# hasindu2008/sigfish

Measured on AMD Instinct MI355X. Metric: reads/s (sDTW alignment stage: nCoV-2019 R9 DNA, -q 250, both strands), higher is better.
Workload: dtype f32

## Files before the change

### include/sigfish_amd.h

```cpp
#ifndef SIGFISH_AMD_H
#define SIGFISH_AMD_H

#include <stddef.h>
#include <stdint.h>

#ifdef __cplusplus
extern "C" {
#endif

#define SFA_VERSION "0.1.0"

#define SFA_RNA 0x001
#define SFA_DTW 0x002
#define SFA_INV 0x004
#define SFA_REF 0x010
#define SFA_END 0x020

enum {
    SFA_OK = 0,
    SFA_EINVAL = -1,
    SFA_ENODEV = -2,
    SFA_ENOMEM = -3,
    SFA_ERANGE = -4,
    SFA_EKERNEL = -5
// ... 21 lines not shown
    uint8_t pad;
} sfa_result_t;

typedef struct {
    uint64_t start;
    float length;
    float mean;
    float stdv;
} sfa_event_t;

typedef struct sfa_ctx sfa_ctx_t;

typedef struct {
    double fill_ms;
    double trace_ms;
    double finalize_ms;
    double total_ms;
    int64_t cells;
    int64_t fill_launches;
    int64_t ckpt_interval;
    int64_t ckpt_bytes;
    int64_t n_tasks;
    int64_t n_chunks;
    int64_t n_segments;
    int64_t segment_reruns;
    double events_ms;
    double normalise_ms;
    int64_t non_finite_reads;
    double decode_ms;
    int64_t blow5_fallbacks;
    int64_t lds_ckpt;
    int64_t trace_margin;
    int64_t fused_trace;
} sfa_profile_t;

typedef struct {
    int32_t n_quads;
    int32_t n_chunks;
    int32_t n_classes;
    int32_t max_rows_per_lane;
    int32_t ckpt_interval;
    int32_t trace_margin;
    int64_t ckpt_bytes;
    int64_t n_tasks;
    int32_t max_lanes_per_read;
    int32_t lane_widening;
} sfa_plan_info_t;

int sfa_init(sfa_ctx_t **ctx, const sfa_ref_t *ref, uint32_t flag, int device);

int sfa_init_devices(sfa_ctx_t **ctx, const sfa_ref_t *ref, uint32_t flag, const int *devices, int n_devices);

int sfa_n_devices(sfa_ctx_t *ctx);

int sfa_align_batch(sfa_ctx_t *ctx, const float *queries, const int64_t *q_off, int32_t n_reads, sfa_result_t *out);

int sfa_align_batch_device(sfa_ctx_t *ctx, const float *d_queries, const int64_t *q_off, int32_t n_reads,
                           sfa_result_t *d_out, int sync);

int sfa_submit_batch(sfa_ctx_t *ctx, const float *queries, const int64_t *q_off, int32_t n_reads);
int sfa_wait_batch(sfa_ctx_t *ctx, sfa_result_t *out, int32_t n_reads);

int sfa_secondary_rows(sfa_ctx_t *ctx, sfa_result_t *sec, int32_t n_reads);

int sfa_event_maps(sfa_ctx_t *ctx, const sfa_result_t *rows, const int32_t *read_of_row, int32_t n_rows, const int64_t *map_off,
                   int32_t *pairs, int32_t *n_on_host);
// ... 119 lines not shown
```

### sigfish_amd/_lib.py

```python
import ctypes as C
import os

HERE = os.path.dirname(os.path.abspath(__file__))
LIB_PATH = os.environ.get("SFA_LIB") or os.path.join(HERE, "lib", "libsigfish_amd.so")

f32p = C.POINTER(C.c_float)
i32p = C.POINTER(C.c_int32)
i64p = C.POINTER(C.c_int64)


class SfaRef(C.Structure):
    _fields_ = [("num_ref", C.c_int32), ("ref_lengths", i32p), ("ref_st_offset", i32p),
                ("forward", C.POINTER(f32p)), ("reverse", C.POINTER(f32p))]


class SfaResult(C.Structure):
    _fields_ = [("rid", C.c_int32), ("pos_st", C.c_int32), ("pos_end", C.c_int32), ("score", C.c_float),
                ("score2", C.c_float), ("strand", C.c_int8), ("mapq", C.c_uint8), ("valid", C.c_uint8),
                ("pad", C.c_uint8)]


class SfaProfile(C.Structure):
    _fields_ = [("fill_ms", C.c_double), ("trace_ms", C.c_double), ("finalize_ms", C.c_double),
                ("total_ms", C.c_double), ("cells", C.c_int64), ("fill_launches", C.c_int64),
                ("ckpt_interval", C.c_int64), ("ckpt_bytes", C.c_int64), ("n_tasks", C.c_int64),
                ("n_chunks", C.c_int64), ("n_segments", C.c_int64), ("segment_reruns", C.c_int64),
                ("events_ms", C.c_double), ("normalise_ms", C.c_double), ("non_finite_reads", C.c_int64), ("decode_ms", C.c_double), ("blow5_fallbacks", C.c_int64), ("lds_ckpt", C.c_int64), ("trace_margin", C.c_int64), ("fused_trace", C.c_int64)]


class SfaPlanInfo(C.Structure):
    _fields_ = [("n_quads", C.c_int32), ("n_chunks", C.c_int32), ("n_classes", C.c_int32),
                ("max_rows_per_lane", C.c_int32), ("ckpt_interval", C.c_int32), ("trace_margin", C.c_int32),
                ("ckpt_bytes", C.c_int64), ("n_tasks", C.c_int64), ("max_lanes_per_read", C.c_int32),
                ("lane_widening", C.c_int32)]


class SfaQueryInfo(C.Structure):
    _fields_ = [("n_events", C.c_int64), ("qstart", C.c_int64), ("qend", C.c_int64), ("start_raw_idx", C.c_uint64),
                ("end_raw_idx", C.c_uint64), ("status", C.c_int32), ("pad", C.c_int32)]


class SfaReadHead(C.Structure):
    _fields_ = [("read_id", C.c_char * 128), ("id_len", C.c_int32), ("pad", C.c_int32), ("n_samples", C.c_int64),
                ("digitisation", C.c_double), ("offset", C.c_double), ("range", C.c_double), ("record_bytes", C.c_int64)]


class SfaEvent(C.Structure):
    _fields_ = [("start", C.c_uint64), ("length", C.c_float), ("mean", C.c_float), ("stdv", C.c_float)]


SYMBOLS = ["sfa_init", "sfa_init_devices", "sfa_n_devices", "sfa_align_batch", "sfa_submit_batch", "sfa_wait_batch", "sfa_align_batch_device", "sfa_align_events", "sfa_align_raw", "sfa_align_raw_ex", "sfa_align_blow5", "sfa_inflate_zlib_device", "sfa_pinned_alloc", "sfa_pinned_free", "sfa_sync",
           "sfa_get_profile", "sfa_stream", "sfa_set_option", "sfa_plan_batch", "sfa_destroy", "sfa_last_error", "sfa_version", "sfa_build_id", "sfa_gen_ref_record",
           "sfa_znormalise", "sfa_paf_row", "sfa_sam_row", "sfa_paf_row_ex", "sfa_sam_row_ex", "sfa_secondary_rows", "sfa_event_maps", "sfa_sam_row_from_map", "sfa_r2qevent_map", "sfa_detect_events", "sfa_select_query", "sfa_detect_query_start", "sfa_set_pore", "sfa_read_kmer_model",
           "sfa_blow5_open", "sfa_blow5_attr", "sfa_blow5_next", "sfa_blow5_close", "sfa_blow5_select_shard", "sfa_blow5_select_records", "sfa_inflate_zlib", "sfa_inflate_zlib_pair", "sfa_device_memory"]

_lib = None


def load():
    global _lib
# ... 80 lines not shown
```

### sigfish_amd/csrc/sdtw_kernels.hpp

```cpp
#pragma once

#include <hip/hip_runtime.h>
#include <stdint.h>

namespace sfa {

constexpr int kRefPad = 128;
#ifndef SFA_STEPS_PER_LOAD
#define SFA_STEPS_PER_LOAD 4
#endif
#ifndef SFA_FILL_WAVES
#define SFA_FILL_WAVES 6
#endif
#ifndef SFA_FILL32_WAVES
#define SFA_FILL32_WAVES 4
#endif
#ifndef SFA_LCK_WAVES
#define SFA_LCK_WAVES 4
#endif
#ifndef SFA_TRACE_WAVES
#define SFA_TRACE_WAVES 4
#endif
constexpr int kStepsPerLoad = SFA_STEPS_PER_LOAD;
constexpr int kSpanBuckets = 32;
// ... 19 lines not shown
    const int32_t *quad_qlen;
    const float *ref;
    const int64_t *job_off;
    const int32_t *job_len;
    const int32_t *chunk_begin;
    const int32_t *job_ck_off;
    float *ck;
    float *p_best;
    int32_t *p_end;
    int32_t *p_job;
    float *p_second;
    int32_t *w_job;
    int32_t *w_end;
    float *w_score;
    ClassDesc cls[kMaxClasses];
    int32_t n_cls;
    int32_t n_chunks;
    int32_t n_tasks;
    int32_t rev_query;
    int32_t ck_shift;
    int32_t trace_margin;
    int32_t n_reads_total;
    int32_t n_seg;
    int32_t warm_windows;
    int32_t n_jobs;
    int32_t verify_planes;
    float *verify;
    int32_t *seg_fail;
    float *best_rec;
    int32_t *best_e;
    unsigned *g_best;
    int32_t *w_chunk;
    int32_t best_planes;
    int32_t coarse_every;
    int32_t lck_shift;
    const struct DpArgs *self;
    unsigned *ticket;
    int32_t *quad_done;
    int32_t n_quads_total;
    const int32_t *job_contig;
    const int8_t *job_strand;
    const int32_t *ref_len;
    const int32_t *ref_st_offset;
    const uint8_t *bad;
    struct ResultRow *out;
    unsigned *span_hist;
    int32_t prio_unit;
    unsigned *started;
    unsigned *err;
    long long spin_limit;
    int32_t debug_drop_quad;
    unsigned long long *task_times;
    int32_t *p_top5;
};

constexpr int kSimdSlots = 16384;
__device__ __forceinline__ unsigned simd_position() {
    const unsigned hw = __builtin_amdgcn_s_getreg((31 << 11) | (0 << 6) | 4);
    const unsigned xcc = __builtin_amdgcn_s_getreg((3 << 11) | (0 << 6) | 20);
    const unsigned simd = (hw >> 4) & 3, cu = (hw >> 8) & 15, sh = (hw >> 12) & 1, se = (hw >> 13) & 7;
    return ((((xcc & 15) * 8 + se) * 2 + sh) * 16 + cu) * 4 + simd;
}

__device__ __forceinline__ void drain_stores() { asm volatile("s_waitcnt vmcnt(0)" ::: "memory"); }
template <int OFF>
__device__ __forceinline__ void store_wt(const float *base, const float v) {
    static_assert(OFF >= 0 && OFF < 4096, "12-bit immediate");
    asm volatile("global_store_dword %0, %1, off offset:%2 sc1" ::"v"(base), "v"(v), "n"(OFF) : "memory");
// ... 230 lines not shown
}

template <int R>
__device__ __forceinline__ void load_query_rows(float (&x)[R], const DpArgs &a, int read, int qlen, int g, int g0 = 0) {
    const float *q = a.queries + a.q_off[read >= 0 ? read : 0];
#pragma unroll
    for (int r = 0; r < R; ++r) {
        const int i = (g - g0) * R + r;
        const int src = a.rev_query ? (qlen - 1 - i) : i;
        x[r] = (read >= 0 && i >= 0 && i < qlen) ? q[src] : 0.0f;
    }
}

struct LdsRows {
    typedef __attribute__((address_space(3))) volatile float lds_vf;
    float *p;
    __device__ __forceinline__ float operator[](const int r) const { return *((lds_vf *)(p + r * 64)); }
    template <int R>
    __device__ __forceinline__ void load(const DpArgs &a, int read, int qlen, int g, int g0) {
        const float *q = a.queries + a.q_off[read >= 0 ? read : 0];
        for (int r = 0; r < R; ++r) {
            const int i = (g - g0) * R + r;
            const int src = a.rev_query ? (qlen - 1 - i) : i;
            *((lds_vf *)(p + r * 64)) = (read >= 0 && i >= 0 && i < qlen) ? q[src] : 0.0f;
        }
    }
};

__device__ __forceinline__ int sweep_begin(int lq) { return lq - ((lq + kStepsPerLoad - 1) & ~(kStepsPerLoad - 1)); }

template <int R>
__device__ __forceinline__ constexpr int ck_planes() { return R + 2; }

constexpr int kLdsCkShift = 9;
constexpr int kLdsCkPlanes = 17;
struct LdsCkpt {
    float *buf;
    int count;
    int e0, e1;
    float *rec;
    int32_t *rec_e;
    unsigned *g_best;
    __device__ __forceinline__ void begin_job() { count = 0; }
    template <int R, typename CV>
    __device__ __forceinline__ void snapshot(const CV &cv, float dprev, int e) {
        count += 1;
        float *b = buf + (count & 1) * (kLdsCkPlanes * 64);
#pragma unroll
        for (int r = 0; r < R; ++r) b[r * 64] = cv[r];
        b[R * 64] = dprev;
        if (count & 1)
            e1 = e;
        else
            e0 = e;
    }
    template <int R, int L, bool WT = false>
    __device__ __forceinline__ void save(unsigned long long improved, float wmin, int e_ws, int margin, int lq, int job, int shift) {
        const int lane = threadIdx.x & 63;
        const int owner_lane = (lane & ~(L - 1)) + lq;
        const bool mine = (improved >> owner_lane) & 1;
        const unsigned wb = __float_as_uint(__shfl(wmin, owner_lane));
        unsigned old = 0;
        if (mine && lane == owner_lane) old = atomicMin(g_best, wb);
        old = __shfl(old, owner_lane);
        if (!(mine && wb <= old)) return;
        const int from = e_ws - margin - 3;
        const int kk = from > 0 ? (from >> shift) : 0;
        if (kk > 0) {
            const float *b = buf + (kk & 1) * (kLdsCkPlanes * 64);
#pragma unroll
            for (int r = 0; r <= R; ++r) {
                if (WT)
                    __hip_atomic_store(rec + r * 64, b[r * 64], __ATOMIC_RELAXED, __HIP_MEMORY_SCOPE_AGENT);
                else
                    rec[r * 64] = b[r * 64];
            }
        }
        if (lane == owner_lane) {
            const int ev = kk > 0 ? ((kk & 1) ? e1 : e0) : -1;
            if (WT)
                __hip_atomic_store(rec_e + lane / L, ev, __ATOMIC_RELAXED, __HIP_MEMORY_SCOPE_AGENT);
            else
                rec_e[lane / L] = ev;
        }
        (void)job;
    }
};

template <int R, bool STD, int RQ, bool LCK = false, int L = 16, bool WT = false, bool SEC = false>
__device__ __forceinline__ void sweep_job(const DpArgs &a, const float *yp, const int rlen, const int qlen, const int lq, const int rq,
                                          const int t_begin, const float (&x)[R], const bool lane0, Exchange &xc, Top2 &top,
                                          const int job, float *ckp, const int T, IssuePriority &pr, const MixedQuad &mq,
                                          LdsCkpt *lck = nullptr, const bool owner = false, int *t5 = nullptr) {
    constexpr bool TRACK = false;
    typename Vec<float, R>::type cv;
    typename Vec<int, R>::type sv;
#pragma unroll
    for (int r = 0; r < R; ++r) {
        cv[r] = INFINITY;
        sv[r] = 0;
    }
    float dprev = INFINITY;
    int sdprev = 0;
    xc.template set_boundary<TRACK>(lane0, 0.0f);

    int e = 0;
    int ck_next = T ? T : 0x7fffffff;
    const int ck_last = T ? ((rlen > 4 ? rlen - 4 : 0) >> a.ck_shift) << a.ck_shift : 0;
    constexpr bool SNAP = LCK && !STD;
    if (SNAP) {
        lck->begin_job();
        ck_next = 1 << a.lck_shift;
    }
    auto maybe_checkpoint = [&]() {
        if (SNAP) {
            if (e >= ck_next) {
                lck->template snapshot<R>(cv, dprev, e);
                ck_next += 1 << a.lck_shift;
                if (T && (lck->count & (a.coarse_every - 1)) == 0 && (lck->count << a.lck_shift) <= ck_last) {
                    if (WT) {
#pragma unroll
                        for (int r = 0; r < R; ++r) __hip_atomic_store(ckp + r * 64, static_cast<float>(cv[r]), __ATOMIC_RELAXED, __HIP_MEMORY_SCOPE_AGENT);
                        __hip_atomic_store(ckp + R * 64, dprev, __ATOMIC_RELAXED, __HIP_MEMORY_SCOPE_AGENT);
                        __hip_atomic_store(ckp + (R + 1) * 64, __int_as_float(e), __ATOMIC_RELAXED, __HIP_MEMORY_SCOPE_AGENT);
                    } else {
#pragma unroll
                        for (int r = 0; r < R; ++r) ckp[r * 64] = cv[r];
                        ckp[R * 64] = dprev;
                        ckp[(R + 1) * 64] = __int_as_float(e);
                    }
                    ckp += ck_planes<R>() * 64;
                }
            }
        } else if (T) {
            if (e >= ck_next && ck_next <= ck_last) {
                if (WT) {
                    store_record_wt<R>(ckp, cv, dprev, e);
                } else {
#pragma unroll
                    for (int r = 0; r < R; ++r) ckp[r * 64] = cv[r];
                    ckp[R * 64] = dprev;
                    ckp[(R + 1) * 64] = __int_as_float(e);
                }
                ckp += ck_planes<R>() * 64;
                ck_next += T;
            }
        }
    };

#define SFA_DP_STEP(YV, U)                                                                                                   \
    do {                                                                                                                     \
        if constexpr (STD) {                                                                                                 \
            if (e >= kStepsPerLoad)                                                                                          \
                dp_step<R, TRACK, STD, int, false>(cv, sv, dprev, sdprev, x, (YV), t_begin + e + (U), lane0, xc);            \
            else                                                                                                             \
                dp_step<R, TRACK, STD, int, true>(cv, sv, dprev, sdprev, x, (YV), t_begin + e + (U), lane0, xc);             \
        } else {                                                                                                             \
            dp_step<R, TRACK, STD, int>(cv, sv, dprev, sdprev, x, (YV), t_begin + e + (U), lane0, xc);                       \
        }                                                                                                                    \
    } while (0)
    float4u ycur = *reinterpret_cast<const float4u *>(yp);
    const int e_main = lq - t_begin;
    for (; e < e_main; e += kStepsPerLoad) {
        const float4u ynext = *reinterpret_cast<const float4u *>(yp + e + kStepsPerLoad);
        maybe_checkpoint();
#pragma unroll
        for (int u = 0; u < kStepsPerLoad; ++u) SFA_DP_STEP(ycur.v[u], u);
        ycur = ynext;
    }
    int jqv = 0;
    constexpr bool MIX = !STD;
    constexpr bool CELL = CellFromFill<R, STD>::value;
    constexpr int NS = 64 / L;
    const int my_slot = (threadIdx.x & 63) / L;
    int q_s[NS], ws_s[NS], we_s[NS];
#pragma unroll
    for (int sl = 0; sl < NS; ++sl) {
        q_s[sl] = MIX ? __builtin_amdgcn_readlane(mq.myq, sl * L) : qlen;
        ws_s[sl] = 0;
        we_s[sl] = min(q_s[sl], rlen);
    }
    float wmin = INFINITY;
    int wpos = CELL ? 0 : -1;
    for (int col = 0; col < rlen;) {
        pr.at_window(col);
        int nxt = we_s[0];
#pragma unroll
        for (int sl = 1; sl < NS; ++sl) nxt = min(nxt, we_s[sl]);
        const int wl = STD ? rlen : nxt - col;
        const int nb = wl >> 2, rm = wl & 3;
        auto track = [&]() {
            const float cl = (RQ >= 0) ? static_cast<float>(cv[RQ >= 0 ? RQ : 0]) : static_cast<float>(cv[rq]);
            if (!CELL) {
                wmin = fminf(wmin, cl);
            } else {
                const bool lt = cl < wmin;
                wmin = lt ? cl : wmin;
                wpos = lt ? jqv : wpos;
                jqv += 1;
            }
        };
        auto block = [&](const float4u &yv) {
            maybe_checkpoint();
#pragma unroll
            for (int u = 0; u < kStepsPerLoad; ++u) {
                SFA_DP_STEP(yv.v[u], u);
                if (!STD) track();
            }
            e += kStepsPerLoad;
        };
        int b = 0;
        for (; R < 32 && b + 1 < nb; b += 2) {
            const float4u yb = *reinterpret_cast<const float4u *>(yp + e + kStepsPerLoad);
            block(ycur);
            ycur = *reinterpret_cast<const float4u *>(yp + e + kStepsPerLoad);
            block(yb);
        }
        for (; b < nb; ++b) {
            const float4u yb = *reinterpret_cast<const float4u *>(yp + e + kStepsPerLoad);
            block(ycur);
            ycur = yb;
        }
        if (rm) {
            const float4u ynext = *reinterpret_cast<const float4u *>(yp + e + rm);
            maybe_checkpoint();
#pragma unroll
            for (int u = 0; u < kStepsPerLoad - 1; ++u) {
                if (u < rm) {
                    SFA_DP_STEP(ycur.v[u], u);
                    if (!STD) track();
                }
            }
            e += rm;
            ycur = ynext;
        }
        if (MIX) {
            unsigned long long endmask = 0;
            int wsl = ws_s[0];
#pragma unroll
            for (int sl = 0; sl < NS; ++sl) {
                const unsigned long long lanes_of_slot = (L == 64) ? ~0ull : (((1ull << (L & 63)) - 1) << ((sl * L) & 63));
                if (we_s[sl] == nxt) endmask |= lanes_of_slot;
                if (sl > 0) wsl = (my_slot == sl) ? ws_s[sl] : wsl;
            }
            const bool ending = (endmask >> (threadIdx.x & 63)) & 1;
            const bool became_best = top.offer_if(ending, wmin, CELL ? wpos : wsl, job);
            if constexpr (SEC) {
                if (ending && owner) top5_offer(t5, wmin, CELL ? wpos : wsl, job);
            }
            if (LCK) {
                const unsigned long long improved = __ballot(became_best && owner);
                if (improved) lck->template save<R, L, WT>(improved, wmin, wsl + e_main, a.trace_margin, lq, job, a.lck_shift);
            }
            wmin = ending ? INFINITY : wmin;
            if (CELL) wpos = ending ? nxt : wpos;
#pragma unroll
            for (int sl = 0; sl < NS; ++sl) {
                if (we_s[sl] == nxt) {
                    ws_s[sl] = nxt;
                    we_s[sl] = min(nxt + q_s[sl], rlen);
                }
            }
        } else {
            const float cl = (RQ >= 0) ? static_cast<float>(cv[RQ >= 0 ? RQ : 0]) : static_cast<float>(cv[rq]);
            top.offer(cl, rlen - 1, job);
            if constexpr (SEC) {
                if (owner) top5_offer(t5, cl, rlen - 1, job);
            }
        }
        col += wl;
    }
    pr.remaining -= rlen;
#undef SFA_DP_STEP
}

template <int R, bool STD, bool LCK = false, int L = 16, bool WT = false, int I = 0, bool SEC = false>
__device__ __forceinline__ void sweep_dispatch(const DpArgs &a, const float *yp, int rlen, int qlen, int lq, int rq, int t_begin,
                                               const float (&x)[R], bool lane0, Exchange &xc, Top2 &top, int job, float *ckp, int T,
                                               IssuePriority &pr, const MixedQuad &mq, LdsCkpt *lck = nullptr, bool owner = false,
                                               int *t5 = nullptr) {
    if constexpr (STD || R > 16) {
        sweep_job<R, STD, -1, LCK, L, WT, SEC>(a, yp, rlen, qlen, lq, rq, t_begin, x, lane0, xc, top, job, ckp, T, pr, mq, lck, owner, t5);
    } else {
        if (rq == I) {
            sweep_job<R, STD, I, LCK, L, WT, SEC>(a, yp, rlen, qlen, lq, rq, t_begin, x, lane0, xc, top, job, ckp, T, pr, mq, lck, owner, t5);
// ... 28 lines not shown

    float x[R];
    load_query_rows<R>(x, a, read, mq.myq, g, mq.g0);
    Exchange xc;
    xc.init(lds_f, lds_i, threadIdx.x >> 6, slot, g, L, mq.g0);

    Top2 top;
    top.init();
    int *t5 = nullptr;
    if constexpr (SEC) {
        t5 = lds_t5 + ((threadIdx.x >> 6) * 4 + slot) * kTop5Words;
        if (g == lq && read >= 0) top5_init(t5);
    }

    const int T = a.ck_shift ? (1 << a.ck_shift) : 0;
    const int64_t ck_total = T ? a.job_ck_off[a.chunk_begin[a.n_chunks]] : 0;

    const int jb = a.chunk_begin[chunk], je = a.chunk_begin[chunk + 1];
    IssuePriority pr;
    {
        int cols = 0;
        const bool on = a.prio_unit > 0;
        if (on)
            for (int job = jb; job < je; ++job) cols += a.job_len[job];
        pr.start(on ? a.prio_unit : 0, cols, FUSED ? a.ticket : a.started, static_cast<unsigned>(a.n_tasks), !FUSED);
    }
    LdsCkpt lck;
    if (LCK && !STD) {
        const int64_t task = static_cast<int64_t>(quad) * a.n_chunks + chunk;
        lck.buf = lds_ck + (threadIdx.x >> 6) * (2 * kLdsCkPlanes * 64) + lane;
        lck.rec = a.best_rec + task * a.best_planes * 64 + lane;
        lck.rec_e = a.best_e + task * 4;
        lck.g_best = a.g_best + (read >= 0 ? read : 0);
        lck.e0 = lck.e1 = 0;
        if (g == lq && read >= 0) {
            if (FUSED)
                __hip_atomic_store(lck.rec_e + slot, -1, __ATOMIC_RELAXED, __HIP_MEMORY_SCOPE_AGENT);
            else
                lck.rec_e[slot] = -1;
        }
    }
    for (int job = jb; job < je; ++job) {
        const int rlen = a.job_len[job];
        const float *yp = a.ref + a.job_off[job] - g + t_begin;
        float *ckp = nullptr;
        if (T) ckp = a.ck + cd.ck_base + (static_cast<int64_t>(quad_local) * ck_total + a.job_ck_off[job]) * (ck_planes<R>() * 64) + lane;
        sweep_dispatch<R, STD, LCK, L, FUSED, 0, SEC>(a, yp, rlen, qlen, lq, rq, t_begin, x, lane0, xc, top, job, ckp, T, pr, mq, &lck, g == lq && read >= 0, t5);
    }

    if (g == lq && read >= 0) {
        const int64_t o = (static_cast<int64_t>(quad) * a.n_chunks + chunk) * 4 + slot;
        if (FUSED) {
            __hip_atomic_store(a.p_best + o, top.best, __ATOMIC_RELAXED, __HIP_MEMORY_SCOPE_AGENT);
            __hip_atomic_store(a.p_second + o, top.second, __ATOMIC_RELAXED, __HIP_MEMORY_SCOPE_AGENT);
            __hip_atomic_store(a.p_end + o, top.end, __ATOMIC_RELAXED, __HIP_MEMORY_SCOPE_AGENT);
            __hip_atomic_store(a.p_job + o, top.job, __ATOMIC_RELAXED, __HIP_MEMORY_SCOPE_AGENT);
        } else {
            a.p_best[o] = top.best;
            a.p_second[o] = top.second;
            a.p_end[o] = top.end;
            a.p_job[o] = top.job;
        }
        if constexpr (SEC) {
            for (int w = 0; w < kTop5Words; ++w) a.p_top5[o * kTop5Words + w] = t5[w];
        }
    }
    if (FUSED) {
// ... 343 lines not shown
    constexpr bool CELL = CellFromFill<R, STD>::value && !LCK;
    const int ws = (read >= 0) ? w.ws : 0;
    const float best = (read >= 0) ? w.best : 0.0f;
    bool done = !(read >= 0 && job >= 0 && ws >= 0);
    job = done ? 0 : job;
    const int rlen = a.job_len[job];
    const int wl = STD ? 1 : min(mq.myq, rlen - ws);
    const int t_begin = sweep_begin(lq);
    const float *ybase = a.ref + a.job_off[job] - g;
    const int t_first = ws + lq;
    const int t_last = CELL ? t_first : ws + wl - 1 + lq;

    const int T = a.ck_shift ? (1 << a.ck_shift) : 0;
    const int64_t ck_total = a.ck_shift ? a.job_ck_off[a.chunk_begin[a.n_chunks]] : 0;
    const int nck = T ? (rlen > 4 ? rlen - 4 : 0) >> a.ck_shift : 0;
    int k = 0;
    if (T) {
        const int from = t_first - a.trace_margin - t_begin - 3;
        k = from > 0 ? (from >> a.ck_shift) : 0;
        k = k < nck ? k : nck;
    }
    int back = 1;
    res_st = -1;
    res_end = -1;
    const unsigned long long owner = __ballot(g == lq);
    bool use_rec = false;
    const float *recp = nullptr;
    int rec_e = -1;
    if (LCK && !STD && !done) {
        const int64_t task = static_cast<int64_t>(quad) * a.n_chunks + w.chunk;
        rec_e = a.best_e[task * 4 + slot];
        recp = a.best_rec + task * a.best_planes * 64 + lane;
        use_rec = rec_e >= 0;
        if (!use_rec) k = 0;
    }

    for (int attempt = 0; attempt < 48; ++attempt) {
        int tb = t_begin;
        typename Vec<float, R>::type c;
        typename Vec<int, R>::type s;
        float dprev;
        int sdprev;
        if (LCK && use_rec) {
#pragma unroll
            for (int r = 0; r < R; ++r) {
                c[r] = recp[r * 64];
                s[r] = -1;
            }
            dprev = recp[R * 64];
            sdprev = -1;
            tb = t_begin + rec_e;
        } else if (k > 0) {
            const float *ckp = a.ck + cd.ck_base +
                               (static_cast<int64_t>(quad_local) * ck_total + a.job_ck_off[job] + (k - 1)) * (ck_planes<R>() * 64) + lane;
#pragma unroll
            for (int r = 0; r < R; ++r) {
                c[r] = ckp[r * 64];
                s[r] = -1;
            }
            dprev = ckp[R * 64];
            sdprev = -1;
            tb = t_begin + __float_as_int(ckp[(R + 1) * 64]);
        } else {
#pragma unroll
            for (int r = 0; r < R; ++r) {
                c[r] = INFINITY;
// ... 18 lines not shown
        for (int tau0 = 0; tau0 < maxlen; tau0 += kStepsPerLoad) {
            const int tbl = min(tb + tau0, tlim);
            const float4u yv = *reinterpret_cast<const float4u *>(ybase + tbl);
#pragma unroll
            for (int u = 0; u < kStepsPerLoad; ++u) {
                const int t = tb + tau0 + u;
                if constexpr (XLDS)
                    dp_step<R, true, STD, int>(c, s, dprev, sdprev, xl, yv.v[u], t - mq.g0, lane0, xc);
                else
                    dp_step<R, true, STD, int>(c, s, dprev, sdprev, x, yv.v[u], t - mq.g0, lane0, xc);
                float cl;
                int sl;
                if constexpr (R >= 32) {
                    pick_row<R>(c, s, rq, cl, sl);
                } else {
                    cl = c[rq];
                    sl = s[rq];
                }
                const bool hit = (cap_end < 0) && !bad_rec && (t >= t_first) && (t <= t_last) && (cl == best);
                cap_end = hit ? (t - lq) : cap_end;
                cap_st = hit ? sl : cap_st;
            }
            if ((__ballot(cap_end >= 0) & owner) == owner) break;
        }
        const int src = (lane & ~(L - 1)) + lq;
        const int q_end = __shfl(cap_end, src), q_st = __shfl(cap_st, src);
        if (!done) {
            if ((q_end >= 0 && q_st >= 0) || (k == 0 && !(LCK && use_rec))) {
                res_end = q_end;
                res_st = q_st;
                done = true;
            } else if (LCK && use_rec) {
                use_rec = false;
            } else {
                k = max(0, k - back);
                back <<= 1;
            }
        }
        if (__all(done)) break;
    }
}

struct ResultRow {
    int32_t rid, pos_st, pos_end;
    float score, score2;
    int8_t strand;
    uint8_t mapq, valid, pad;
};

struct FinalizeArgs {
    const int32_t *slot_of_read;
    const float *p_best;
    const int32_t *p_end;
    const int32_t *p_job;
    const float *p_second;
    const int32_t *job_contig;
    const int8_t *job_strand;
    const int32_t *ref_len;
    const int32_t *ref_st_offset;
    int32_t *w_job;
    int32_t *w_end;
    float *w_score;
    int32_t *w_chunk;
    const int32_t *t_st;
    ResultRow *out;
    const uint8_t *bad;
// ... 379 lines not shown
```

### sigfish_amd/csrc/sfa_align.hip

```cpp
#include "sfa_ctx.hpp"
#define SFA_DEFINE_FINALIZE_KERNEL
#include "sdtw_kernels.hpp"
#include "sdtw_instances.hpp"
#include "sdtw_strips.hpp"

using sfa::DpArgs;
using sfa::FinalizeArgs;
using sfa::Route;
using sfa::SecArgs;
using sfa::ResultRow;
using sfa::align_device;
using sfa::for_each_shard;
using sfa::for_each_shard_range;
using sfa::resolve_profile;

namespace {

static_assert(sizeof(ResultRow) == sizeof(sfa_result_t), "result row layout");

template <int Cap, typename F>
void by_rows(int maxr, F f) {
    if constexpr (Cap >= 32) {
        if (maxr >= 32) return f(std::integral_constant<int, 32>());
    }
// ... 168 lines not shown
    }
    if (two_sets) {
        HIP_TRY(hipEventRecord(c->lev[3], c->stream_long2));
        HIP_TRY(hipStreamWaitEvent(first, c->lev[3], 0));
    }
    return SFA_OK;
}


int align_sliced(sfa_ctx *c, const float *d_queries, const int64_t *q_off, int32_t n, ResultRow *d_out, ResultRow *d_sec, int32_t slices) {
    sfa_profile_t sum{};
    for (int32_t s = 0; s < slices; ++s) {
        const int32_t lo = static_cast<int32_t>(static_cast<int64_t>(n) * s / slices);
        const int32_t hi = static_cast<int32_t>(static_cast<int64_t>(n) * (s + 1) / slices);
        c->in_slice = true;
        int rc = align_device(c, d_queries, q_off + lo, hi - lo, d_out + lo, d_sec ? d_sec + 4 * static_cast<int64_t>(lo) : nullptr);
        c->in_slice = false;
        if (rc) return rc;
        if ((rc = resolve_profile(c))) return rc;
        sum.fill_ms += c->prof.fill_ms;
        sum.trace_ms += c->prof.trace_ms;
        sum.finalize_ms += c->prof.finalize_ms;
        sum.total_ms += c->prof.total_ms;
        sum.cells += c->prof.cells;
        sum.fill_launches += c->prof.fill_launches;
        sum.ckpt_interval = std::max(sum.ckpt_interval, c->prof.ckpt_interval);
        sum.ckpt_bytes = std::max(sum.ckpt_bytes, c->prof.ckpt_bytes);
        sum.trace_margin = std::max(sum.trace_margin, c->prof.trace_margin);
        sum.lds_ckpt = std::max(sum.lds_ckpt, c->prof.lds_ckpt);
        sum.fused_trace = std::max(sum.fused_trace, c->prof.fused_trace);
        sum.n_tasks += c->prof.n_tasks;
        sum.n_chunks = std::max(sum.n_chunks, c->prof.n_chunks);
        sum.non_finite_reads += c->prof.non_finite_reads;
    }
    c->prof = sum;
    return SFA_OK;
}


bool fused(Route r) { return r == Route::LdsFused || r == Route::Fused32; }
bool lds(Route r) { return r == Route::Lds || r == Route::LdsFused; }

sfa::PlanParams plan_params(const sfa_ctx *c) {
    sfa::PlanParams pp;
    pp.n_sims = static_cast<int64_t>(c->cu_count) * 4;
    pp.waves_per_simd = c->opt_waves_per_simd;
    pp.ckpt_interval = c->opt_ckpt_interval;
    pp.ckpt_budget_bytes = c->opt_ckpt_budget;
    pp.trace_margin = c->opt_trace_margin;
    pp.lane_widening = c->opt_lane_widening;
    pp.widen_below = c->opt_widen_below;
    pp.column_segments = c->opt_column_segments;
    pp.segment_warm_windows = c->opt_segment_warm;
    pp.std_dtw = (c->flag & SFA_DTW) != 0;
    pp.span_sixteenths = c->span_sixteenths;
    pp.allow_segments = !pp.std_dtw && !c->no_segments_once && c->opt_secondary == 0;
    pp.lds_ckpt = c->opt_secondary > 0 ? 0 : static_cast<int>(c->opt_lds_ckpt);
    return pp;
}

struct LongReads {
    std::vector<int32_t> reads;
    int64_t events = 0, max = 0;
};

struct Staging {
// ... 77 lines not shown
    da.p_best = c->d_pbest.as<float>();
    da.p_end = c->d_pend.as<int32_t>();
    da.p_job = c->d_pjob.as<int32_t>();
    da.p_second = c->d_psecond.as<float>();
    da.w_job = c->d_wjob.as<int32_t>();
    da.w_end = c->d_wend.as<int32_t>();
    da.w_score = c->d_wscore.as<float>();
    da.n_reads_total = n;
    da.n_cls = static_cast<int32_t>(plan.classes.size());
    for (int i = 0; i < da.n_cls; ++i) {
        da.cls[i].R = plan.classes[i].R;
        da.cls[i].lanes = plan.classes[i].lanes;
        da.cls[i].quad_base = plan.classes[i].quad_base;
        da.cls[i].n_quads = plan.classes[i].n_quads;
        da.cls[i].task_base = plan.classes[i].quad_base * n_chunks;
        da.cls[i].ck_base = plan.classes[i].ck_base;
    }
    da.n_chunks = n_chunks;
    da.n_tasks = n_quads * n_chunks;
    da.rev_query = ((c->flag & SFA_RNA) && !(c->flag & SFA_INV)) ? 1 : 0;
    da.ck_shift = plan.ck_shift;
    da.trace_margin = plan.trace_margin;
    da.n_seg = plan.n_seg;
    da.warm_windows = plan.warm_windows;
    da.n_jobs = n_jobs;
    da.verify_planes = plan.max_R + 1;
    da.verify = c->d_verify.as<float>();
    da.seg_fail = c->d_segfail.as<int32_t>();
    da.best_rec = c->d_bestrec.as<float>();
    da.best_e = c->d_beste.as<int32_t>();
    da.g_best = c->d_gbest.as<unsigned>();
    da.w_chunk = c->d_wchunk.as<int32_t>();
    da.best_planes = sfa::kLdsCkPlanes;
    da.lck_shift = plan.lck_shift;
    da.coarse_every = (lds(route) && plan.ck_shift >= plan.lck_shift) ? (1 << (plan.ck_shift - plan.lck_shift)) : 1;
    da.ticket = c->d_ticket.as<unsigned>();
    da.quad_done = c->d_quaddone.as<int32_t>();
    da.n_quads_total = n_quads;
    da.job_contig = c->d_job_contig.as<int32_t>();
    da.job_strand = c->d_job_strand.as<int8_t>();
    da.ref_len = c->d_ref_len.as<int32_t>();
    da.ref_st_offset = c->d_ref_off.as<int32_t>();
    da.bad = c->d_bad.as<uint8_t>();
    da.out = d_out;
    da.span_hist = route == Route::Fused32 ? c->d_badcount.as<unsigned>() + 8 : nullptr;
    da.prio_unit = static_cast<int32_t>(c->opt_prio_unit);
    da.started = c->d_started.as<unsigned>();
    da.err = c->d_badcount.as<unsigned>() + 4;
    {
        int64_t longest = 0;
        for (int32_t ch = 0; ch < n_chunks; ++ch) {
            int64_t cols = 0;
            for (int32_t j = plan.chunk_begin[ch]; j < plan.chunk_begin[ch + 1] && j < n_jobs; ++j) cols += c->h_job_len[j];
            longest = std::max(longest, cols);
        }
        da.spin_limit = std::max<int64_t>(c->opt_spin_limit_ms, longest / 1000) * 100000;
        c->quad_limit_ms = da.spin_limit / 100000;
    }
    da.debug_drop_quad = static_cast<int32_t>(c->opt_debug_drop_quad);
    da.p_top5 = route == Route::Secondary ? c->d_p5.as<int32_t>() : nullptr;
    da.self = fused(route) ? c->d_args.as<DpArgs>() : nullptr;
#ifdef SFA_TASK_TIMES
    da.task_times = c->d_times.as<unsigned long long>();
#endif

    FinalizeArgs &fz = a.fz;
    fz.slot_of_read = reinterpret_cast<const int32_t *>(ds + sg.slot);
    fz.p_best = da.p_best;
    fz.p_end = da.p_end;
    fz.p_job = da.p_job;
    fz.p_second = da.p_second;
    fz.job_contig = da.job_contig;
    fz.job_strand = da.job_strand;
    fz.ref_len = da.ref_len;
    fz.ref_st_offset = da.ref_st_offset;
    fz.w_job = da.w_job;
    fz.w_end = da.w_end;
    fz.w_score = da.w_score;
    fz.w_chunk = da.w_chunk;
    fz.t_st = c->d_tst.as<int32_t>();
    fz.out = d_out;
// ... 236 lines not shown
    HIP_TRY(hipEventSynchronize(c->ev[4]));
    float a = 0, b = 0, d = 0, t = 0;
    HIP_TRY(hipEventElapsedTime(&a, c->ev[0], c->ev[1]));
    HIP_TRY(hipEventElapsedTime(&b, c->ev[1], c->ev[2]));
    HIP_TRY(hipEventElapsedTime(&d, c->ev[2], c->ev[3]));
    HIP_TRY(hipEventElapsedTime(&t, c->ev[0], c->ev[4]));
    if (c->prof.fused_trace) d = 0;
    if (c->long_pending) {
        float l = 0;
        HIP_TRY(hipEventElapsedTime(&l, c->ev[5], c->ev[4]));
        a += l;
        a = t;
        d = 0;
        c->long_pending = false;
    }
    c->prof.events_ms = c->prof.normalise_ms = 0;
    c->prof.decode_ms = 0;
    c->prof.blow5_fallbacks = c->blow5_fallbacks;
    if (c->bev_pending) {
        float d1 = 0;
        HIP_TRY(hipEventElapsedTime(&d1, c->bev[0], c->bev[1]));
        c->prof.decode_ms = d1;
        c->bev_pending = false;
    }
    if (c->eev_pending) {
        float e1 = 0, e2 = 0;
        HIP_TRY(hipEventElapsedTime(&e1, c->eev[0], c->eev[1]));
        HIP_TRY(hipEventElapsedTime(&e2, c->eev[2], c->eev[3]));
        c->prof.events_ms = e1;
        c->prof.normalise_ms = e2;
        c->eev_pending = false;
    }
    c->prof.non_finite_reads = c->h_badcount.p ? *c->h_badcount.as<unsigned>() : 0;
    c->prof.fill_ms = a;
    c->prof.trace_ms = d;
    c->prof.finalize_ms = t - a - d;
    c->prof.total_ms = t;
    c->prof_pending = false;
    if (c->h_badcount.p) {
        const unsigned *e = c->h_badcount.as<unsigned>() + 4;
        if (e[0] == sfa::kErrQuadWait)
            return fail(SFA_EKERNEL, "fused launch: pass 2 of quad %u waited %lld ms for its fill tasks (%u of them had completed); rows of this batch are invalid",
                        e[1], (long long)c->quad_limit_ms, e[2]);
        if (e[0] == sfa::kErrStripWait)
            return fail(SFA_EKERNEL, "row strips: a strip waited %lld ms for column %u of the row above (column %u was published); rows of this batch are invalid",
                        (long long)c->strip_limit_ms, e[1], e[2]);
        if (e[0]) return fail(SFA_EKERNEL, "device error word %u (%u, %u)", e[0], e[1], e[2]);
    }
    if (c->h_badcount.p) {
        const unsigned *h = c->h_badcount.as<unsigned>() + 8;
        uint64_t total = 0;
        for (int b = 0; b < sfa::kSpanBuckets; ++b) total += h[b];
        if (total >= 64) {
            uint64_t acc = 0;
            int b = 0;
            for (; b < sfa::kSpanBuckets; ++b) {
                acc += h[b];
                if (acc * 1000 >= total * 999) break;
            }
            c->span_sixteenths = std::min(16, b + 2);
        }
    }
    return SFA_OK;
}

extern "C" {
// ... 155 lines not shown
```

### sigfish_amd/csrc/sfa_context.hip

```cpp
#include "sfa_ctx.hpp"
#include "sdtw_kernels.hpp"

namespace sfa {
std::string &last_error_slot() {
    thread_local std::string err;
    return err;
}
}
using sfa::resolve_profile;

extern "C" {

const char *sfa_last_error(void) { return sfa::last_error_slot().c_str(); }
void sfa_set_error_(const char *msg) { sfa::last_error_slot() = msg ? msg : ""; }
const char *sfa_version(void) { return SFA_VERSION; }
#ifndef SFA_BUILD_ID
#define SFA_BUILD_ID "unknown"
#endif
const char *sfa_build_id(void) { return SFA_BUILD_ID; }

}

struct HostRef {
    int32_t num_ref = 0, n_jobs = 0;
// ... 273 lines not shown
int sfa_sync(sfa_ctx_t *c) {
    if (!c) return fail(SFA_EINVAL, "null context");
    if (!c->shards.empty()) {
        for (sfa_ctx *sh : c->shards)
            if (int rc = sfa_sync(sh)) return rc;
        return SFA_OK;
    }
    HIP_TRY(hipSetDevice(c->device));
    HIP_TRY(hipStreamSynchronize(c->stream));
    return resolve_profile(c);
}

int sfa_get_profile(sfa_ctx_t *c, sfa_profile_t *p) {
    if (!c || !p) return fail(SFA_EINVAL, "null argument");
    if (!c->shards.empty()) {
        sfa_profile_t sum{};
        for (sfa_ctx *sh : c->shards) {
            sfa_profile_t q;
            if (int rc = sfa_get_profile(sh, &q)) return rc;
            sum.fill_ms = std::max(sum.fill_ms, q.fill_ms);
            sum.trace_ms = std::max(sum.trace_ms, q.trace_ms);
            sum.finalize_ms = std::max(sum.finalize_ms, q.finalize_ms);
            sum.total_ms = std::max(sum.total_ms, q.total_ms);
            sum.events_ms = std::max(sum.events_ms, q.events_ms);
            sum.decode_ms = std::max(sum.decode_ms, q.decode_ms);
            sum.blow5_fallbacks += q.blow5_fallbacks;
            sum.normalise_ms = std::max(sum.normalise_ms, q.normalise_ms);
            sum.cells += q.cells;
            sum.fill_launches += q.fill_launches;
            sum.n_tasks += q.n_tasks;
            sum.ckpt_bytes += q.ckpt_bytes;
            sum.segment_reruns += q.segment_reruns;
            sum.non_finite_reads += q.non_finite_reads;
            sum.ckpt_interval = std::max(sum.ckpt_interval, q.ckpt_interval);
            sum.n_chunks = std::max(sum.n_chunks, q.n_chunks);
            sum.n_segments = std::max(sum.n_segments, q.n_segments);
            sum.lds_ckpt = std::max(sum.lds_ckpt, q.lds_ckpt);
            sum.fused_trace = std::max(sum.fused_trace, q.fused_trace);
            sum.trace_margin = std::max(sum.trace_margin, q.trace_margin);
        }
        *p = sum;
        return SFA_OK;
    }
    if (int rc = resolve_profile(c)) return rc;
    *p = c->prof;
    return SFA_OK;
}

void *sfa_stream(sfa_ctx_t *c) { return (c && c->shards.empty()) ? static_cast<void *>(c->stream) : nullptr; }

int sfa_n_devices(sfa_ctx_t *c) { return !c ? 0 : (c->shards.empty() ? 1 : static_cast<int>(c->shards.size())); }

#ifdef SFA_TASK_TIMES
int64_t sfa_debug_task_times(sfa_ctx_t *c, unsigned long long *out, int64_t cap_tasks) {
    if (!c || !out) return -1;
    if (hipSetDevice(c->device) != hipSuccess || hipStreamSynchronize(c->stream) != hipSuccess) return -1;
    const int64_t n = std::min<int64_t>(cap_tasks, c->n_times);
    if (n > 0 && hipMemcpy(out, c->d_times.p, 24 * static_cast<size_t>(n), hipMemcpyDeviceToHost) != hipSuccess) return -1;
    return n;
}
int64_t sfa_debug_task_times_long(sfa_ctx_t *c, unsigned long long *out, int64_t cap_tasks) {
    if (!c || !out) return -1;
    if (hipSetDevice(c->device) != hipSuccess || hipDeviceSynchronize() != hipSuccess) return -1;
    const int64_t n = std::min<int64_t>(cap_tasks, c->n_ltimes);
    if (n > 0 && hipMemcpy(out, c->d_ltimes.p, 24 * static_cast<size_t>(n), hipMemcpyDeviceToHost) != hipSuccess) return -1;
    return n;
// ... 5 lines not shown
```

### sigfish_amd/csrc/sfa_plan.hpp

```cpp
#pragma once

#include <algorithm>
#include <cstdint>
#include <string>
#include <vector>

namespace sfa {

constexpr int kMaxQuery = 2048;

struct ClassShape {
    int R, lanes;
};
constexpr ClassShape kClassShapes[6] = {{32, 64}, {32, 32}, {32, 16}, {16, 16}, {8, 16}, {4, 16}};

inline ClassShape widened(int ci, int w) {
    ClassShape s = kClassShapes[ci];
    while (w > 1 && s.lanes < 64 && s.R > 4) {
        s.R /= 2;
        s.lanes *= 2;
        w /= 2;
    }
    return s;
}
// ... 1 lines not shown
inline int class_for(int qlen) {
    if (qlen > kMaxQuery) return -1;
    int c = 0;
    while (c + 1 < 6 && qlen <= kClassShapes[c + 1].R * kClassShapes[c + 1].lanes) ++c;
    return c;
}

inline int64_t ck_count(int32_t rlen, int shift) { return (rlen > 4 ? rlen - 4 : 0) >> shift; }

struct PlanParams {
    int64_t n_sims = 1024;
    int64_t waves_per_simd = 6;
    int64_t ckpt_interval = 0;
    int64_t ckpt_budget_bytes = 32ll << 30;
    int64_t trace_margin = -1;
    int32_t span_sixteenths = 0;
    int64_t lane_widening = 0;
    int64_t widen_below = 5;
    int64_t column_segments = 0;
    int64_t segment_warm_windows = 4;
    bool allow_segments = true;
    int lds_ckpt = 0;
    bool std_dtw = false;
    bool skip_long = false;
};

struct PlanClass {
    int R = 0, lanes = 16, quad_base = 0, n_quads = 0;
    int64_t ck_base = 0;
};

struct BatchPlan {
    int32_t n_quads = 0, n_chunks = 1, max_R = 4, max_lanes = 16, widening = 1, ck_shift = 0, trace_margin = 0;
    int32_t lck_shift = 9;
    int32_t n_seg = 1, warm_windows = 4;
    bool lds_ckpt = false;
    int64_t ck_floats = 0, query_events = 0;
    std::vector<int32_t> order;
    std::vector<int32_t> quad_qlen;
    std::vector<int32_t> slot_of_read;
    std::vector<int32_t> chunk_begin;
    std::vector<int32_t> job_ck_off;
    std::vector<PlanClass> classes;
    std::vector<int32_t> s_qlen, s_count, s_fill_pos, s_slot_start, s_len_quad_base;
    std::vector<int8_t> s_per_shift;
    void reset() {
        n_quads = 0; n_chunks = 1; max_R = 4; max_lanes = 16; widening = 1; ck_shift = 0; trace_margin = 0; lck_shift = 9;
        n_seg = 1; warm_windows = 4;
        lds_ckpt = false;
        ck_floats = 0; query_events = 0;
        classes.clear();
    }
};

inline void split_jobs(const std::vector<int32_t> &job_len, int64_t total_cols, int32_t n_chunks, int32_t *chunk_begin) {
    const int32_t n_jobs = static_cast<int32_t>(job_len.size());
    int64_t acc = 0;
    int32_t j = 0;
    chunk_begin[0] = 0;
    for (int32_t ch = 1; ch < n_chunks; ++ch) {
        const int64_t want = total_cols * ch / n_chunks;
        acc += job_len[j++];
        while (j < n_jobs - (n_chunks - ch) && acc + job_len[j] / 2 < want) acc += job_len[j++];
        chunk_begin[ch] = j;
    }
    chunk_begin[n_chunks] = n_jobs;
}

inline int plan_batch(const int64_t *q_off, int32_t n, const std::vector<int32_t> &job_len, int64_t total_cols,
                      const PlanParams &pp, BatchPlan *out, std::string *err) {
    BatchPlan &p = *out;
    p.reset();
    const int32_t n_jobs = static_cast<int32_t>(job_len.size());
    std::vector<int32_t> &qlen = p.s_qlen, &count = p.s_count, &fill_pos = p.s_fill_pos;
    qlen.assign(n, 0);
    count.assign(kMaxQuery + 2, 0);
    int maxq = 0;
    for (int32_t i = 0; i < n; ++i) {
        const int64_t l = q_off[i + 1] - q_off[i];
        if (l < 0) {
// ... 87 lines not shown
        const int32_t qd = len_quad_base[l] + (k >> sh);
        const int32_t sl = qd * 4 + (k & ((1 << sh) - 1));
        p.order[sl] = i;
        p.slot_of_read[i] = sl;
        p.quad_qlen[qd] = std::max(p.quad_qlen[qd], l);
    }
    if (n_quads == 0) p.quad_qlen[0] = 1;

    if (pp.allow_segments && p.widening == 4 && p.max_lanes == 64 && n_quads > 0) {
        int32_t min_len = n_jobs ? job_len[0] : 0;
        for (int32_t j = 1; j < n_jobs; ++j) min_len = std::min(min_len, job_len[j]);
        const int64_t tasks = static_cast<int64_t>(n_quads) * n_jobs;
        int64_t S = pp.column_segments > 0 ? pp.column_segments : ((pp.widen_below + 1) * pp.n_sims + tasks - 1) / tasks;
        S = std::min<int64_t>(S, 64);
        S = std::min<int64_t>(S, min_len / (4 * std::max<int64_t>(pp.segment_warm_windows, 1) * std::max(maxq, 1)));
        if (S >= 3 || (pp.column_segments > 1 && S >= 2)) p.n_seg = static_cast<int32_t>(S);
        p.warm_windows = static_cast<int32_t>(pp.segment_warm_windows);
    }
    if (p.n_seg > 1) {
        p.n_chunks = n_jobs * p.n_seg;
        p.chunk_begin.resize(p.n_chunks + 1);
        for (int32_t c = 0; c < p.n_chunks; ++c) p.chunk_begin[c] = c / p.n_seg;
        p.chunk_begin[p.n_chunks] = n_jobs;
    } else {
        p.n_chunks = chunks_for(n_quads);
        p.chunk_begin.resize(p.n_chunks + 1);
        split_jobs(job_len, total_cols, p.n_chunks, p.chunk_begin.data());
    }

    p.job_ck_off.assign(n_jobs + 1, 0);
    p.trace_margin = static_cast<int32_t>(pp.trace_margin >= 0 ? pp.trace_margin : maxq + p.max_lanes);
    const bool adapt = pp.trace_margin < 0 && pp.span_sixteenths > 0;
    p.lds_ckpt = pp.lds_ckpt && pp.ckpt_interval == 0 && p.max_R <= 16 && p.n_seg == 1 && n_quads > 0 && maxq <= (pp.lds_ckpt >= 2 ? 1024 : 256);
    p.lck_shift = maxq <= 256 ? 9 : (maxq <= 512 ? 10 : 11);
    {
        const int64_t tasks = static_cast<int64_t>(n_quads) * p.n_chunks;
        if (pp.lds_ckpt < 2 && tasks > 4 * pp.n_sims && tasks <= 6 * pp.n_sims) p.lds_ckpt = false;
    }
    if (p.lds_ckpt && !pp.std_dtw) p.trace_margin = std::min<int32_t>(p.trace_margin, (1 << p.lck_shift) - maxq - 3);
    if (adapt && !p.lds_ckpt && !pp.std_dtw)
        p.trace_margin = std::min<int32_t>(p.trace_margin, static_cast<int32_t>((static_cast<int64_t>(maxq) * pp.span_sixteenths) / 16) + p.max_lanes + 16);
    if (n_quads > 0) {
        int shift = p.lds_ckpt ? 15 : 9;
        if (pp.ckpt_interval > 0) {
            shift = 0;
            while ((1ll << shift) < pp.ckpt_interval) ++shift;
        }
        for (;; ++shift) {
            int64_t per_quad = 0;
            for (int32_t j = 0; j < n_jobs; ++j) per_quad += ck_count(job_len[j], shift);
            int64_t floats = 0;
            for (const PlanClass &cl : p.classes) floats += per_quad * cl.n_quads * (cl.R + 2) * 64;
            if (pp.ckpt_interval > 0 || floats * 4 <= pp.ckpt_budget_bytes || per_quad == 0 || shift >= 30) {
                p.ck_shift = shift;
                p.ck_floats = floats;
                break;
            }
        }
        int64_t base = 0, per_quad = 0;
        for (int32_t j = 0; j < n_jobs; ++j) {
            p.job_ck_off[j] = static_cast<int32_t>(per_quad);
            per_quad += ck_count(job_len[j], p.ck_shift);
        }
        p.job_ck_off[n_jobs] = static_cast<int32_t>(per_quad);
        for (PlanClass &cl : p.classes) {
            cl.ck_base = base;
            base += per_quad * cl.n_quads * (cl.R + 2) * 64;
        }
    }
    return 0;
}

// ... 60 lines not shown
```

Before: 1.298 million.

## Snapshot LDS checkpoints at per-lane window ends instead of fixed intervals

```diff
diff --git a/include/sigfish_amd.h b/include/sigfish_amd.h
--- a/include/sigfish_amd.h
+++ b/include/sigfish_amd.h
@@ -77,6 +77,8 @@
     int64_t lds_ckpt;
     int64_t trace_margin;
     int64_t fused_trace;
+    int64_t lck_fallbacks;
+    int64_t lck_from_scratch;
 } sfa_profile_t;
 
 typedef struct {
diff --git a/sigfish_amd/_lib.py b/sigfish_amd/_lib.py
--- a/sigfish_amd/_lib.py
+++ b/sigfish_amd/_lib.py
@@ -25,7 +25,7 @@
                 ("total_ms", C.c_double), ("cells", C.c_int64), ("fill_launches", C.c_int64),
                 ("ckpt_interval", C.c_int64), ("ckpt_bytes", C.c_int64), ("n_tasks", C.c_int64),
                 ("n_chunks", C.c_int64), ("n_segments", C.c_int64), ("segment_reruns", C.c_int64),
-                ("events_ms", C.c_double), ("normalise_ms", C.c_double), ("non_finite_reads", C.c_int64), ("decode_ms", C.c_double), ("blow5_fallbacks", C.c_int64), ("lds_ckpt", C.c_int64), ("trace_margin", C.c_int64), ("fused_trace", C.c_int64)]
+                ("events_ms", C.c_double), ("normalise_ms", C.c_double), ("non_finite_reads", C.c_int64), ("decode_ms", C.c_double), ("blow5_fallbacks", C.c_int64), ("lds_ckpt", C.c_int64), ("trace_margin", C.c_int64), ("fused_trace", C.c_int64), ("lck_fallbacks", C.c_int64), ("lck_from_scratch", C.c_int64)]
 
 
 class SfaPlanInfo(C.Structure):
diff --git a/sigfish_amd/csrc/sdtw_kernels.hpp b/sigfish_amd/csrc/sdtw_kernels.hpp
--- a/sigfish_amd/csrc/sdtw_kernels.hpp
+++ b/sigfish_amd/csrc/sdtw_kernels.hpp
@@ -75,8 +75,7 @@
     unsigned *g_best;
     int32_t *w_chunk;
     int32_t best_planes;
-    int32_t coarse_every;
-    int32_t lck_shift;
+    unsigned *lck_stats;
     const struct DpArgs *self;
     unsigned *ticket;
     int32_t *quad_done;
@@ -373,30 +372,27 @@
 template <int R>
 __device__ __forceinline__ constexpr int ck_planes() { return R + 2; }
 
-constexpr int kLdsCkShift = 9;
 constexpr int kLdsCkPlanes = 17;
 struct LdsCkpt {
     float *buf;
-    int count;
-    int e0, e1;
+    unsigned long long par;
     float *rec;
     int32_t *rec_e;
     unsigned *g_best;
-    __device__ __forceinline__ void begin_job() { count = 0; }
+    __device__ __forceinline__ void begin_job() { par = 0; }
     template <int R, typename CV>
-    __device__ __forceinline__ void snapshot(const CV &cv, float dprev, int e) {
-        count += 1;
-        float *b = buf + (count & 1) * (kLdsCkPlanes * 64);
-#pragma unroll
-        for (int r = 0; r < R; ++r) b[r * 64] = cv[r];
-        b[R * 64] = dprev;
-        if (count & 1)
-            e1 = e;
-        else
-            e0 = e;
+    __device__ __forceinline__ void snapshot(const unsigned long long endmask, const CV &cv, const float dprev) {
+        const int lane = threadIdx.x & 63;
+        if ((endmask >> lane) & 1) {
+            float *b = buf + static_cast<int>((par >> lane) & 1) * (kLdsCkPlanes * 64);
+#pragma unroll
+            for (int r = 0; r < R; ++r) b[r * 64] = cv[r];
+            b[R * 64] = dprev;
+        }
+        par ^= endmask;
     }
     template <int R, int L, bool WT = false>
-    __device__ __forceinline__ void save(unsigned long long improved, float wmin, int e_ws, int margin, int lq, int job, int shift) {
+    __device__ __forceinline__ void save(unsigned long long improved, float wmin, int ws, int myq, int e_main, int lq) {
         const int lane = threadIdx.x & 63;
         const int owner_lane = (lane & ~(L - 1)) + lq;
         const bool mine = (improved >> owner_lane) & 1;
@@ -405,10 +401,9 @@
         if (mine && lane == owner_lane) old = atomicMin(g_best, wb);
         old = __shfl(old, owner_lane);
         if (!(mine && wb <= old)) return;
-        const int from = e_ws - margin - 3;
-        const int kk = from > 0 ? (from >> shift) : 0;
-        if (kk > 0) {
-            const float *b = buf + (kk & 1) * (kLdsCkPlanes * 64);
+        const bool have = ws >= 2 * myq;
+        if (have) {
+            const float *b = buf + static_cast<int>((par >> lane) & 1) * (kLdsCkPlanes * 64);
 #pragma unroll
             for (int r = 0; r <= R; ++r) {
                 if (WT)
@@ -418,13 +413,12 @@
             }
         }
         if (lane == owner_lane) {
-            const int ev = kk > 0 ? ((kk & 1) ? e1 : e0) : -1;
+            const int ev = have ? e_main + ws - myq : -1;
             if (WT)
                 __hip_atomic_store(rec_e + lane / L, ev, __ATOMIC_RELAXED, __HIP_MEMORY_SCOPE_AGENT);
             else
                 rec_e[lane / L] = ev;
         }
-        (void)job;
     }
 };
 
@@ -449,31 +443,9 @@
     int ck_next = T ? T : 0x7fffffff;
     const int ck_last = T ? ((rlen > 4 ? rlen - 4 : 0) >> a.ck_shift) << a.ck_shift : 0;
     constexpr bool SNAP = LCK && !STD;
-    if (SNAP) {
-        lck->begin_job();
-        ck_next = 1 << a.lck_shift;
-    }
+    if (SNAP) lck->begin_job();
     auto maybe_checkpoint = [&]() {
-        if (SNAP) {
-            if (e >= ck_next) {
-                lck->template snapshot<R>(cv, dprev, e);
-                ck_next += 1 << a.lck_shift;
-                if (T && (lck->count & (a.coarse_every - 1)) == 0 && (lck->count << a.lck_shift) <= ck_last) {
-                    if (WT) {
-#pragma unroll
-                        for (int r = 0; r < R; ++r) __hip_atomic_store(ckp + r * 64, static_cast<float>(cv[r]), __ATOMIC_RELAXED, __HIP_MEMORY_SCOPE_AGENT);
-                        __hip_atomic_store(ckp + R * 64, dprev, __ATOMIC_RELAXED, __HIP_MEMORY_SCOPE_AGENT);
-                        __hip_atomic_store(ckp + (R + 1) * 64, __int_as_float(e), __ATOMIC_RELAXED, __HIP_MEMORY_SCOPE_AGENT);
-                    } else {
-#pragma unroll
-                        for (int r = 0; r < R; ++r) ckp[r * 64] = cv[r];
-                        ckp[R * 64] = dprev;
-                        ckp[(R + 1) * 64] = __int_as_float(e);
-                    }
-                    ckp += ck_planes<R>() * 64;
-                }
-            }
-        } else if (T) {
+        if (!SNAP && T) {
             if (e >= ck_next && ck_next <= ck_last) {
                 if (WT) {
                     store_record_wt<R>(ckp, cv, dprev, e);
@@ -530,6 +502,23 @@
         for (int sl = 1; sl < NS; ++sl) nxt = min(nxt, we_s[sl]);
         const int wl = STD ? rlen : nxt - col;
         const int nb = wl >> 2, rm = wl & 3;
+        if (SNAP && T) {
+            while (e + wl > ck_next && ck_next <= ck_last) {
+                if (WT) {
+#pragma unroll
+                    for (int r = 0; r < R; ++r) __hip_atomic_store(ckp + r * 64, static_cast<float>(cv[r]), __ATOMIC_RELAXED, __HIP_MEMORY_SCOPE_AGENT);
+                    __hip_atomic_store(ckp + R * 64, dprev, __ATOMIC_RELAXED, __HIP_MEMORY_SCOPE_AGENT);
+                    __hip_atomic_store(ckp + (R + 1) * 64, __int_as_float(e), __ATOMIC_RELAXED, __HIP_MEMORY_SCOPE_AGENT);
+                } else {
+#pragma unroll
+                    for (int r = 0; r < R; ++r) ckp[r * 64] = cv[r];
+                    ckp[R * 64] = dprev;
+                    ckp[(R + 1) * 64] = __int_as_float(e);
+                }
+                ckp += ck_planes<R>() * 64;
+                ck_next += T;
+            }
+        }
         auto track = [&]() {
             const float cl = (RQ >= 0) ? static_cast<float>(cv[RQ >= 0 ? RQ : 0]) : static_cast<float>(cv[rq]);
             if (!CELL) {
@@ -589,9 +578,10 @@
             if constexpr (SEC) {
                 if (ending && owner) top5_offer(t5, wmin, CELL ? wpos : wsl, job);
             }
-            if (LCK) {
+            if (SNAP) {
                 const unsigned long long improved = __ballot(became_best && owner);
-                if (improved) lck->template save<R, L, WT>(improved, wmin, wsl + e_main, a.trace_margin, lq, job, a.lck_shift);
+                if (improved) lck->template save<R, L, WT>(improved, wmin, wsl, mq.myq, e_main, lq);
+                lck->template snapshot<R>(endmask, cv, dprev);
             }
             wmin = ending ? INFINITY : wmin;
             if (CELL) wpos = ending ? nxt : wpos;
@@ -686,7 +676,6 @@
         lck.rec = a.best_rec + task * a.best_planes * 64 + lane;
         lck.rec_e = a.best_e + task * 4;
         lck.g_best = a.g_best + (read >= 0 ? read : 0);
-        lck.e0 = lck.e1 = 0;
         if (g == lq && read >= 0) {
             if (FUSED)
                 __hip_atomic_store(lck.rec_e + slot, -1, __ATOMIC_RELAXED, __HIP_MEMORY_SCOPE_AGENT);
@@ -1096,6 +1085,7 @@
         rec_e = a.best_e[task * 4 + slot];
         recp = a.best_rec + task * a.best_planes * 64 + lane;
         use_rec = rec_e >= 0;
+        if (!use_rec && g == lq) atomicAdd(a.lck_stats + 1, 1u);
         if (!use_rec) k = 0;
     }
 
@@ -1180,6 +1170,7 @@
                 done = true;
             } else if (LCK && use_rec) {
                 use_rec = false;
+                if (g == lq) atomicAdd(a.lck_stats, 1u);
             } else {
                 k = max(0, k - back);
                 back <<= 1;
diff --git a/sigfish_amd/csrc/sfa_align.hip b/sigfish_amd/csrc/sfa_align.hip
--- a/sigfish_amd/csrc/sfa_align.hip
+++ b/sigfish_amd/csrc/sfa_align.hip
@@ -224,6 +224,8 @@
         sum.n_tasks += c->prof.n_tasks;
         sum.n_chunks = std::max(sum.n_chunks, c->prof.n_chunks);
         sum.non_finite_reads += c->prof.non_finite_reads;
+        sum.lck_fallbacks += c->prof.lck_fallbacks;
+        sum.lck_from_scratch += c->prof.lck_from_scratch;
     }
     c->prof = sum;
     return SFA_OK;
@@ -367,8 +369,6 @@
     da.g_best = c->d_gbest.as<unsigned>();
     da.w_chunk = c->d_wchunk.as<int32_t>();
     da.best_planes = sfa::kLdsCkPlanes;
-    da.lck_shift = plan.lck_shift;
-    da.coarse_every = (lds(route) && plan.ck_shift >= plan.lck_shift) ? (1 << (plan.ck_shift - plan.lck_shift)) : 1;
     da.ticket = c->d_ticket.as<unsigned>();
     da.quad_done = c->d_quaddone.as<int32_t>();
     da.n_quads_total = n_quads;
@@ -382,6 +382,7 @@
     da.prio_unit = static_cast<int32_t>(c->opt_prio_unit);
     da.started = c->d_started.as<unsigned>();
     da.err = c->d_badcount.as<unsigned>() + 4;
+    da.lck_stats = c->d_badcount.as<unsigned>() + 2;
     {
         int64_t longest = 0;
         for (int32_t ch = 0; ch < n_chunks; ++ch) {
@@ -684,6 +685,8 @@
         c->eev_pending = false;
     }
     c->prof.non_finite_reads = c->h_badcount.p ? *c->h_badcount.as<unsigned>() : 0;
+    c->prof.lck_fallbacks = c->h_badcount.p ? c->h_badcount.as<unsigned>()[2] : 0;
+    c->prof.lck_from_scratch = c->h_badcount.p ? c->h_badcount.as<unsigned>()[3] : 0;
     c->prof.fill_ms = a;
     c->prof.trace_ms = d;
     c->prof.finalize_ms = t - a - d;
diff --git a/sigfish_amd/csrc/sfa_context.hip b/sigfish_amd/csrc/sfa_context.hip
--- a/sigfish_amd/csrc/sfa_context.hip
+++ b/sigfish_amd/csrc/sfa_context.hip
@@ -329,6 +329,8 @@
             sum.ckpt_bytes += q.ckpt_bytes;
             sum.segment_reruns += q.segment_reruns;
             sum.non_finite_reads += q.non_finite_reads;
+            sum.lck_fallbacks += q.lck_fallbacks;
+            sum.lck_from_scratch += q.lck_from_scratch;
             sum.ckpt_interval = std::max(sum.ckpt_interval, q.ckpt_interval);
             sum.n_chunks = std::max(sum.n_chunks, q.n_chunks);
             sum.n_segments = std::max(sum.n_segments, q.n_segments);
diff --git a/sigfish_amd/csrc/sfa_plan.hpp b/sigfish_amd/csrc/sfa_plan.hpp
--- a/sigfish_amd/csrc/sfa_plan.hpp
+++ b/sigfish_amd/csrc/sfa_plan.hpp
@@ -57,7 +57,6 @@
 
 struct BatchPlan {
     int32_t n_quads = 0, n_chunks = 1, max_R = 4, max_lanes = 16, widening = 1, ck_shift = 0, trace_margin = 0;
-    int32_t lck_shift = 9;
     int32_t n_seg = 1, warm_windows = 4;
     bool lds_ckpt = false;
     int64_t ck_floats = 0, query_events = 0;
@@ -70,7 +69,7 @@
     std::vector<int32_t> s_qlen, s_count, s_fill_pos, s_slot_start, s_len_quad_base;
     std::vector<int8_t> s_per_shift;
     void reset() {
-        n_quads = 0; n_chunks = 1; max_R = 4; max_lanes = 16; widening = 1; ck_shift = 0; trace_margin = 0; lck_shift = 9;
+        n_quads = 0; n_chunks = 1; max_R = 4; max_lanes = 16; widening = 1; ck_shift = 0; trace_margin = 0;
         n_seg = 1; warm_windows = 4;
         lds_ckpt = false;
         ck_floats = 0; query_events = 0;
@@ -224,12 +223,11 @@
     p.trace_margin = static_cast<int32_t>(pp.trace_margin >= 0 ? pp.trace_margin : maxq + p.max_lanes);
     const bool adapt = pp.trace_margin < 0 && pp.span_sixteenths > 0;
     p.lds_ckpt = pp.lds_ckpt && pp.ckpt_interval == 0 && p.max_R <= 16 && p.n_seg == 1 && n_quads > 0 && maxq <= (pp.lds_ckpt >= 2 ? 1024 : 256);
-    p.lck_shift = maxq <= 256 ? 9 : (maxq <= 512 ? 10 : 11);
     {
         const int64_t tasks = static_cast<int64_t>(n_quads) * p.n_chunks;
         if (pp.lds_ckpt < 2 && tasks > 4 * pp.n_sims && tasks <= 6 * pp.n_sims) p.lds_ckpt = false;
     }
-    if (p.lds_ckpt && !pp.std_dtw) p.trace_margin = std::min<int32_t>(p.trace_margin, (1 << p.lck_shift) - maxq - 3);
+    if (p.lds_ckpt && !pp.std_dtw) p.trace_margin = std::min<int32_t>(p.trace_margin, maxq - (maxq - 1) / p.max_R);
     if (adapt && !p.lds_ckpt && !pp.std_dtw)
         p.trace_margin = std::min<int32_t>(p.trace_margin, static_cast<int32_t>((static_cast<int64_t>(maxq) * pp.span_sixteenths) / 16) + p.max_lanes + 16);
     if (n_quads > 0) {
```

After: 1.346 million, median of 6. 3.6% higher.
